# fabiocarrara/neural-ode-features

Measured on AMD Instinct MI355X. Metric: images/sec (fwd+adjoint) CIFAR-10 ODE-ResNet bs=128 at 1/2/4/8 GPU, higher is better.
Workload: dtype f32

## Files before the change

include/node_hip.h:

```cpp
#ifndef NODE_HIP_H
#define NODE_HIP_H

#include <stddef.h>
#include <stdint.h>

#ifdef __cplusplus
extern "C" {
#endif

#define NODE_ABI_VERSION 6

enum { NODE_METHOD_DOPRI5 = 0, NODE_METHOD_RK4 = 1 };

enum {
  NODE_OK = 0,
  NODE_ERR_NULL = -1,
  NODE_ERR_SHAPE = -2,
  NODE_ERR_UNSUPPORTED = -3,
  NODE_ERR_WORKSPACE = -4,
  NODE_ERR_MAX_STEPS = -5,
  NODE_ERR_NONFINITE = -6,
  NODE_ERR_DT_UNDERFLOW = -7,
  NODE_ERR_HIP = -8,
  NODE_ERR_ARG = -9
// ... 216 lines not shown
  const float* b1_n2_b;
  const float* b1_c2_w;
  const float* b1_ds_w;
  const float* b2_n1_w;
  const float* b2_n1_b;
  const float* b2_c1_w;
  const float* b2_n2_w;
  const float* b2_n2_b;
  const float* b2_c2_w;
  const float* b2_ds_w;
} node_stem_params;
typedef struct node_stem_grads {
  float* conv0_w; float* conv0_b;
  float* b1_n1_w; float* b1_n1_b; float* b1_c1_w; float* b1_n2_w; float* b1_n2_b; float* b1_c2_w; float* b1_ds_w;
  float* b2_n1_w; float* b2_n1_b; float* b2_c1_w; float* b2_n2_w; float* b2_n2_b; float* b2_c2_w; float* b2_ds_w;
} node_stem_grads;
size_t node_stem_workspace_bytes(const node_stem_shape* shape);
int node_stem_fwd(const node_stem_shape* shape, const node_stem_params* params, const float* x, float* out,
                  void* ws, size_t ws_bytes, void* stream);
int node_stem_bwd(const node_stem_shape* shape, const node_stem_params* params, const float* x, const float* grad_out,
                  const node_stem_grads* grads, void* ws, size_t ws_bytes, void* stream);
int node_stem_bwd_dx(const node_stem_shape* shape, const node_stem_params* params, const float* x, const float* grad_out,
                     const node_stem_grads* grads, float* d_x, void* ws, size_t ws_bytes, void* stream);
size_t node_stem_conv0_dgrad_workspace_bytes(const node_stem_shape* shape);
int node_stem_conv0_dgrad(const node_stem_shape* shape, const float* w0, const float* dy, float* d_x,
                          void* ws, size_t ws_bytes, void* stream);

typedef struct node_conv_geom {
  int32_t n, cin, cout, x_h, x_w, k, stride, pad;
} node_conv_geom;
size_t node_stem_conv_workspace_bytes(const node_conv_geom* g);
int node_stem_conv(const node_conv_geom* g, int what, const float* x, const float* w, const float* dy, float* result,
                   void* ws, size_t ws_bytes, void* stream);

typedef struct node_trunk_shape {
  int32_t n, channels, h, w, blocks;
  float eps;
} node_trunk_shape;
typedef struct node_trunk_block {
  const float* n1_w;
  const float* n1_b;
  const float* c1_w;
  const float* n2_w;
  const float* n2_b;
  const float* c2_w;
} node_trunk_block;
typedef struct node_trunk_block_grads {
  float* n1_w; float* n1_b; float* c1_w; float* n2_w; float* n2_b; float* c2_w;
} node_trunk_block_grads;
size_t node_trunk_workspace_bytes(const node_trunk_shape* shape, int keep_for_backward);
int node_trunk_fwd(const node_trunk_shape* shape, const node_trunk_block* blocks, const float* x, float* out, float* taps,
                   int keep_for_backward, void* ws, size_t ws_bytes, void* stream);
int node_trunk_bwd(const node_trunk_shape* shape, const node_trunk_block* blocks, const float* grad_out,
                   const node_trunk_block_grads* grads, float* d_x, void* ws, size_t ws_bytes, void* stream);

size_t node_retrieval_workspace_bytes(int nq, int nd, int d);
int node_retrieval_ap(int nq, int nd, int d, const float* q, const float* x, const int32_t* q_labels, const int32_t* x_labels,
                      int k, double* ap, double* ap_k, void* ws, size_t ws_bytes, void* stream);
int node_rank_ap(int nq, int nd, const float* scores, const int32_t* q_labels, const int32_t* x_labels, int k, double* ap,
                 double* ap_k, void* ws, size_t ws_bytes, void* stream);

typedef struct { int32_t fold; int32_t cls; float c; } node_svm_problem;
typedef struct { int32_t iterations; int32_t converged; double grad_ratio; } node_svm_result;
size_t node_svm_workspace_bytes(int n, int d, int p);
int node_svm_fit(int n, int d, int p, const float* x, const int32_t* labels, const int32_t* row_fold,
                 const node_svm_problem* problems, double eps, int max_iter, float* weights, node_svm_result* results, void* ws,
// ... 56 lines not shown
```

neural-ode-features_amd/_lib.py:

```python
from __future__ import annotations

import ctypes as C
import os

HERE = os.path.dirname(os.path.abspath(__file__))
LIB_PATH = os.path.join(HERE, 'csrc', 'libnode_hip.so')
LIB_DIAG_PATH = os.path.join(HERE, 'csrc', 'libnode_hip_diag.so')

NODE_ABI_VERSION = 6
METHOD_DOPRI5, METHOD_RK4 = 0, 1
METHODS = {'dopri5': METHOD_DOPRI5, 'rk4': METHOD_RK4}

ERRORS = {
    0: 'NODE_OK', -1: 'NODE_ERR_NULL', -2: 'NODE_ERR_SHAPE', -3: 'NODE_ERR_UNSUPPORTED',
    -4: 'NODE_ERR_WORKSPACE', -5: 'NODE_ERR_MAX_STEPS', -6: 'NODE_ERR_NONFINITE',
    -7: 'NODE_ERR_DT_UNDERFLOW', -8: 'NODE_ERR_HIP', -9: 'NODE_ERR_ARG',
}

EXPORTS = [
    'node_abi_version', 'node_last_error', 'node_param_count', 'node_workspace_bytes', 'node_solve_is_resident',
    'node_describe_dims',
    'node_odefunc_fwd', 'node_odefunc_vjp', 'node_solve_fwd', 'node_solve_adjoint',
    'node_backprop_workspace_bytes', 'node_solve_backprop',
    'node_head_fwd', 'node_head_bwd', 'node_gn_relu_fwd', 'node_gn_relu_bwd',
    'node_sgd_step', 'node_adam_step', 'node_profile_begin', 'node_profile_end',
    'node_conv3x3_w4_workspace_bytes', 'node_conv3x3_w4', 'node_w4_split3', 'node_w4_pair_stats',
    'node_stem_workspace_bytes', 'node_stem_fwd', 'node_stem_bwd', 'node_stem_conv_workspace_bytes', 'node_stem_conv',
    'node_stem_bwd_dx', 'node_stem_conv0_dgrad_workspace_bytes', 'node_stem_conv0_dgrad', 'node_attack_step', 'node_attack_judge',
    'node_head_loss_scratch_bytes', 'node_head_loss_fwd', 'node_head_loss_bwd',
    'node_flat_workspace_bytes', 'node_flat_begin', 'node_flat_stage', 'node_flat_scalar', 'node_flat_initial_step',
    'node_flat_finish_step', 'node_flat_status_read',
    'node_retrieval_workspace_bytes', 'node_retrieval_ap', 'node_rank_ap',
    'node_svm_workspace_bytes', 'node_svm_fit', 'node_svm_cv_score',
    'node_augment_batch',
    'node_imgconv_workspace_bytes', 'node_imgconv_fwd', 'node_imgconv_bwd',
    'node_trunk_workspace_bytes', 'node_trunk_fwd', 'node_trunk_bwd',
]


class NodeShape(C.Structure):
    _fields_ = [('n', C.c_int32), ('c', C.c_int32), ('h', C.c_int32), ('w', C.c_int32),
                ('groups', C.c_int32), ('eps', C.c_float)]


class NodeParams(C.Structure):
    _fields_ = [(k, C.c_void_p) for k in (
        'norm1_w', 'norm1_b', 'conv1_w', 'conv1_b', 'norm2_w', 'norm2_b',
        'conv2_w', 'conv2_b', 'norm3_w', 'norm3_b')]


WGRAD_KERNELS = ('W2_8', 'W2_4', 'W_8_8', 'W_16_2', 'W_4_4', 'T_8_8', 'T_16_4', 'T_7_7', 'T_4_4', 'P')
CONV_KERNELS = ('DIRECT_64', 'DIRECT_128', 'DIRECT_256', 'W1_64', 'W1_128', 'W1_256', 'W2_128')


class NodeDimsInfo(C.Structure):
    _fields_ = [(k, C.c_int32) for k in (
        'wgrad_kernel', 'conv_kernel', 'wino', 'bm', 's', 'csplit', 'mtiles', 'ntile', 'small', 'tiny', 'wino4', 'w4q',
        'wgrad_wino', 'wut', 'rb', 'nbands', 'nsplit', 'wgrad_pair')]


def describe_dims(n, c, h, w, groups=None, eps=1e-5):
# ... 42 lines not shown

class NodeAdamTensor(C.Structure):
    _fields_ = [('param', C.c_void_p), ('grad', C.c_void_p), ('exp_avg', C.c_void_p), ('exp_avg_sq', C.c_void_p),
                ('step', C.c_void_p), ('n', C.c_size_t)]


STEM_PARAM_FIELDS = ('conv0_w', 'conv0_b', 'b1_n1_w', 'b1_n1_b', 'b1_c1_w', 'b1_n2_w', 'b1_n2_b', 'b1_c2_w', 'b1_ds_w',
                     'b2_n1_w', 'b2_n1_b', 'b2_c1_w', 'b2_n2_w', 'b2_n2_b', 'b2_c2_w', 'b2_ds_w')


class NodeStemShape(C.Structure):
    _fields_ = [('n', C.c_int32), ('in_ch', C.c_int32), ('h', C.c_int32), ('w', C.c_int32), ('filters', C.c_int32),
                ('eps', C.c_float)]


class NodeStemParams(C.Structure):
    _fields_ = [(k, C.c_void_p) for k in STEM_PARAM_FIELDS]


TRUNK_BLOCK_FIELDS = ('n1_w', 'n1_b', 'c1_w', 'n2_w', 'n2_b', 'c2_w')


class NodeTrunkShape(C.Structure):
    _fields_ = [('n', C.c_int32), ('channels', C.c_int32), ('h', C.c_int32), ('w', C.c_int32), ('blocks', C.c_int32),
                ('eps', C.c_float)]


class NodeTrunkBlock(C.Structure):
    _fields_ = [(k, C.c_void_p) for k in TRUNK_BLOCK_FIELDS]


class NodeConvGeom(C.Structure):
    _fields_ = [(k, C.c_int32) for k in ('n', 'cin', 'cout', 'x_h', 'x_w', 'k', 'stride', 'pad')]


REDUCE_MEAN, REDUCE_SUM = 0, 1


class NodeHeadLoss(C.Structure):
    _fields_ = [('n', C.c_int32), ('c', C.c_int32), ('classes', C.c_int32), ('reduction', C.c_int32),
                ('pooled', C.c_void_p), ('weight', C.c_void_p), ('bias', C.c_void_p), ('target', C.c_void_p),
                ('logits', C.c_void_p), ('loss', C.c_void_p), ('stat', C.c_void_p), ('scratch', C.c_void_p)]


class NodeHeadLossGrad(C.Structure):
    _fields_ = [(k, C.c_void_p) for k in ('grad_loss', 'grad_logits', 'd_logits', 'd_pooled', 'd_weight', 'd_bias')]


class NodeFlatSeg(C.Structure):
    _fields_ = [('y', C.c_void_p), ('y1', C.c_void_p), ('k', C.c_void_p * 7), ('n', C.c_size_t)]


class NodeFlatSolve(C.Structure):
    _fields_ = [('nseg', C.c_int32), ('has_scalar', C.c_int32), ('seg', NodeFlatSeg * 3), ('rtol', C.c_float), ('atol', C.c_float),
                ('tsign', C.c_float), ('n_targets', C.c_int32), ('ws', C.c_void_p), ('ws_bytes', C.c_size_t)]


class NodeFlatStatus(C.Structure):
    _fields_ = [('done', C.c_int32), ('status', C.c_int32), ('steps', C.c_int32), ('accepted', C.c_int32), ('rejected', C.c_int32),
                ('t', C.c_double), ('dt', C.c_double), ('first_dt', C.c_double), ('scalar', C.c_float)]


FLAT_F0, FLAT_PROBE = -1, -2

AUG_CROP, AUG_JITTER, AUG_FLIP, AUG_NORM = 1, 2, 4, 8

# ... 75 lines not shown
    lib.node_head_fwd.argtypes = [P(NodeShape), vp, vp, vp, vp, vp, vp, vp]
    lib.node_head_bwd.restype = i32
    lib.node_head_bwd.argtypes = [P(NodeShape), vp, vp, vp, vp, vp, vp, vp, vp, vp, vp]
    lib.node_gn_relu_fwd.restype = i32
    lib.node_gn_relu_fwd.argtypes = [P(NodeShape), vp, vp, vp, i32, vp, vp, vp]
    lib.node_gn_relu_bwd.restype = i32
    lib.node_gn_relu_bwd.argtypes = [P(NodeShape), vp, vp, vp, vp, i32, vp, vp, vp, vp, vp]
    lib.node_sgd_step.restype = i32
    lib.node_sgd_step.argtypes = [P(NodeSgdTensor), i32, f32, f32, f32, f32, vp, vp]
    lib.node_adam_step.restype = i32
    lib.node_adam_step.argtypes = [P(NodeAdamTensor), i32, f32, f32, f32, f32, f32, f32, vp, vp]
    lib.node_profile_begin.restype = i32
    lib.node_profile_begin.argtypes = []
    lib.node_profile_end.restype = i32
    lib.node_profile_end.argtypes = [P(NodeProfile)]
    lib.node_conv3x3_w4_workspace_bytes.restype = sz
    lib.node_conv3x3_w4_workspace_bytes.argtypes = [P(NodeShape)]
    lib.node_w4_pair_stats.restype = i32
    lib.node_w4_pair_stats.argtypes = [P(C.c_int32)]
    lib.node_conv3x3_w4.restype = i32
    lib.node_conv3x3_w4.argtypes = [P(NodeShape), vp, i32, vp, vp, vp, sz, vp]
    lib.node_w4_split3.restype = i32
    lib.node_w4_split3.argtypes = [vp, vp, sz, vp]
    lib.node_stem_workspace_bytes.restype = sz
    lib.node_stem_workspace_bytes.argtypes = [P(NodeStemShape)]
    lib.node_stem_fwd.restype = i32
    lib.node_stem_fwd.argtypes = [P(NodeStemShape), P(NodeStemParams), vp, vp, vp, sz, vp]
    lib.node_stem_bwd.restype = i32
    lib.node_stem_bwd.argtypes = [P(NodeStemShape), P(NodeStemParams), vp, vp, P(NodeStemParams), vp, sz, vp]
    lib.node_stem_conv_workspace_bytes.restype = sz
    lib.node_stem_conv_workspace_bytes.argtypes = [P(NodeConvGeom)]
    lib.node_stem_conv.restype = i32
    lib.node_stem_conv.argtypes = [P(NodeConvGeom), i32, vp, vp, vp, vp, vp, sz, vp]
    lib.node_stem_bwd_dx.restype = i32
    lib.node_stem_bwd_dx.argtypes = [P(NodeStemShape), P(NodeStemParams), vp, vp, P(NodeStemParams), vp, vp, sz, vp]
    lib.node_stem_conv0_dgrad_workspace_bytes.restype = sz
    lib.node_stem_conv0_dgrad_workspace_bytes.argtypes = [P(NodeStemShape)]
    lib.node_stem_conv0_dgrad.restype = i32
    lib.node_stem_conv0_dgrad.argtypes = [P(NodeStemShape), vp, vp, vp, vp, sz, vp]
    lib.node_attack_step.restype = i32
    lib.node_attack_step.argtypes = [P(NodeAttack), vp, vp, vp, vp, vp, vp]
    lib.node_attack_judge.restype = i32
    lib.node_attack_judge.argtypes = [P(NodeAttack), i32, vp, vp, vp, vp, i32, i32, P(NodeAttackRecord), vp]
    lib.node_head_loss_scratch_bytes.restype = sz
    lib.node_head_loss_scratch_bytes.argtypes = [i32]
    lib.node_head_loss_fwd.restype = i32
    lib.node_head_loss_fwd.argtypes = [P(NodeHeadLoss), vp]
    lib.node_head_loss_bwd.restype = i32
    lib.node_head_loss_bwd.argtypes = [P(NodeHeadLoss), P(NodeHeadLossGrad), vp]
    lib.node_flat_workspace_bytes.restype = sz
    lib.node_flat_workspace_bytes.argtypes = [i32]
    lib.node_flat_begin.restype = i32
    lib.node_flat_begin.argtypes = [P(NodeFlatSolve), C.c_double, P(C.c_double), C.c_double, i32, vp]
    lib.node_flat_stage.restype = i32
    lib.node_flat_stage.argtypes = [P(NodeFlatSolve), i32, i32, P(C.c_void_p), vp, vp]
    lib.node_flat_scalar.restype = i32
    lib.node_flat_scalar.argtypes = [P(NodeFlatSolve), i32, vp, f32, i32, vp]
    lib.node_flat_initial_step.restype = i32
    lib.node_flat_initial_step.argtypes = [P(NodeFlatSolve), i32, vp]
    lib.node_flat_finish_step.restype = i32
    lib.node_flat_finish_step.argtypes = [P(NodeFlatSolve), i32, vp, vp]
    lib.node_flat_status_read.restype = i32
    lib.node_flat_status_read.argtypes = [P(NodeFlatSolve), P(NodeFlatStatus), vp]
    lib.node_retrieval_workspace_bytes.restype = sz
    lib.node_retrieval_workspace_bytes.argtypes = [i32, i32, i32]
    lib.node_retrieval_ap.restype = i32
# ... 34 lines not shown
```

neural-ode-features_amd/csrc/kernels_stem.hip:

```cpp
#include "stem.h"
#include <type_traits>

namespace node {

namespace {

typedef float f32x16 __attribute__((ext_vector_type(16)));
typedef __bf16 bf16x8 __attribute__((ext_vector_type(8)));
typedef __bf16 bf16x2 __attribute__((ext_vector_type(2)));
typedef float f32x2 __attribute__((ext_vector_type(2)));
typedef unsigned u32x4 __attribute__((ext_vector_type(4)));

__device__ __forceinline__ void split3(float x, bf16_t& h, bf16_t& m, bf16_t& l) {
  const __bf16 bh = (__bf16)x;
  const float r = x - (float)bh;
  const __bf16 bm = (__bf16)r;
  const float r2 = r - (float)bm;
  const __bf16 bl = (__bf16)r2;
  h = __builtin_bit_cast(bf16_t, bh);
  m = __builtin_bit_cast(bf16_t, bm);
  l = __builtin_bit_cast(bf16_t, bl);
}
__device__ __forceinline__ void split8(const float4& p, const float4& q, u32x4& hh, u32x4& mm, u32x4& ll) {
  const f32x2 v[4] = {{p.x, p.y}, {p.z, p.w}, {q.x, q.y}, {q.z, q.w}};
#pragma unroll
  for (int i = 0; i < 4; ++i) {
    const bf16x2 h = __builtin_convertvector(v[i], bf16x2);
    const f32x2 r = v[i] - __builtin_convertvector(h, f32x2);
    const bf16x2 m = __builtin_convertvector(r, bf16x2);
    const f32x2 r2 = r - __builtin_convertvector(m, f32x2);
    const bf16x2 l = __builtin_convertvector(r2, bf16x2);
    hh[i] = __builtin_bit_cast(unsigned, h);
    mm[i] = __builtin_bit_cast(unsigned, m);
// ... 544 lines not shown
    } else {
#pragma unroll
      for (int q = 0; q < 8; ++q) av[q] = make_float4(0.f, 0.f, 0.f, 0.f);
    }
    f32x16 acc;
#pragma unroll
    for (int i = 0; i < 16; ++i) acc[i] = 0.f;
#pragma unroll
    for (int q = 0; q < 8; ++q) {
      acc = __builtin_amdgcn_mfma_f32_32x32x2f32(av[q].x, b[4 * q], acc, 0, 0, 0);
      acc = __builtin_amdgcn_mfma_f32_32x32x2f32(av[q].y, b[4 * q + 1], acc, 0, 0, 0);
      acc = __builtin_amdgcn_mfma_f32_32x32x2f32(av[q].z, b[4 * q + 2], acc, 0, 0, 0);
      acc = __builtin_amdgcn_mfma_f32_32x32x2f32(av[q].w, b[4 * q + 3], acc, 0, 0, 0);
    }
    if (li < 28) {
#pragma unroll
      for (int i = 0; i < 16; ++i) P[(tile * 32 + 8 * (i >> 2) + 4 * hh + (i & 3)) * DG_PS + li] = acc[i];
    }
  }
  __syncthreads();
  for (int idx = t; idx < Cin * DG_TH * DG_TW; idx += 256) {
    const int xx = idx % DG_TW, yy = (idx / DG_TW) % DG_TH, ci = idx / (DG_TW * DG_TH);
    const int y = y0 + yy, x = x0 + xx;
    if (y >= H || x >= W) continue;
    float s = 0.f;
#pragma unroll
    for (int ky = 0; ky < 3; ++ky)
#pragma unroll
      for (int kx = 0; kx < 3; ++kx) s += P[((yy + 2 - ky) * DG_PW + xx + 2 - kx) * DG_PS + ci * 9 + ky * 3 + kx];
    dx[((size_t)(n * Cin + ci) * H + y) * W + x] = s;
  }
}

__device__ __forceinline__ void group_sums(float v, float* red, float* grp, int CB, int cpg, int t) {
  red[t] = v;
  __syncthreads();
  const int ngrp = CB / cpg;
  if (t < ngrp) {
    float s = 0.f;
    for (int j = 0; j < 256 / CB; ++j)
      for (int k = 0; k < cpg; ++k) s += red[j * CB + t * cpg + k];
    grp[t] = s;
  }
  __syncthreads();
}

__global__ __launch_bounds__(256) void k_stem_gn_fwd(const SGnArgs a) {
  extern __shared__ __align__(16) unsigned char smem[];
  const int t = threadIdx.x;
  const int CB = a.CB, HW = a.HW, C = a.C;
  float* tile = reinterpret_cast<float*>(smem);
  float* red = tile + (size_t)HW * CB;
  float* gmean = red + 256;
  float* grstd = gmean + 128;
  const int nblk = C / CB;
  const int n = blockIdx.x / nblk, c0 = (blockIdx.x - n * nblk) * CB;
  const int q4 = CB >> 2;
  const float* src = a.h + ((size_t)n * HW) * C + c0;
  for (int idx = t; idx < HW * q4; idx += 256) {
    const int px = idx / q4, q = idx - px * q4;
    *reinterpret_cast<float4*>(tile + px * CB + 4 * q) = *reinterpret_cast<const float4*>(src + (size_t)px * C + 4 * q);
  }
  __syncthreads();
  const int c = t & (CB - 1), pg = t / CB, PG = 256 / CB;
  const float inv_m = 1.f / (float)(a.cpg * HW);
  float s = 0.f;
  for (int px = pg; px < HW; px += PG) s += tile[px * CB + c];
  group_sums(s, red, gmean, CB, a.cpg, t);
  const float mean = gmean[c / a.cpg] * inv_m;
  float s2 = 0.f;
  for (int px = pg; px < HW; px += PG) {
    const float d = tile[px * CB + c] - mean;
    s2 += d * d;
  }
  group_sums(s2, red, grstd, CB, a.cpg, t);
  const int ngrp = CB / a.cpg;
  if (t < ngrp) {
    const float m = gmean[t] * inv_m, rs = rsqrtf(grstd[t] * inv_m + a.eps);
    float* st = a.stats + ((size_t)n * (C / a.cpg) + c0 / a.cpg + t) * 2;
    st[0] = m;
    st[1] = rs;
  }
  __syncthreads();
  if (t < ngrp) {
    const float m = gmean[t] * inv_m, rs = rsqrtf(grstd[t] * inv_m + a.eps);
    gmean[t] = m;
    grstd[t] = rs;
  }
  __syncthreads();
  const int q8 = CB >> 3;
  for (int idx = t; idx < HW * q8; idx += 256) {
    const int px = idx / q8, q = idx - px * q8;
    const float4 p0 = *reinterpret_cast<const float4*>(tile + px * CB + 8 * q);
    const float4 p1 = *reinterpret_cast<const float4*>(tile + px * CB + 8 * q + 4);
    float v[8] = {p0.x, p0.y, p0.z, p0.w, p1.x, p1.y, p1.z, p1.w};
#pragma unroll
    for (int k = 0; k < 8; ++k) {
      const int cc = 8 * q + k, g = cc / a.cpg;
      const float y = (v[k] - gmean[g]) * grstd[g] * a.gamma[c0 + cc] + a.beta[c0 + cc];
      v[k] = fmaxf(y, 0.f);
    }
    u32x4 hh, mm, ll;
    split8(make_float4(v[0], v[1], v[2], v[3]), make_float4(v[4], v[5], v[6], v[7]), hh, mm, ll);
    bf16_t* dst = a.a3 + ((size_t)n * HW + px) * C + c0 + 8 * q;
    *reinterpret_cast<u32x4*>(dst) = hh;
    *reinterpret_cast<u32x4*>(dst + a.a_plane) = mm;
    *reinterpret_cast<u32x4*>(dst + 2 * a.a_plane) = ll;
  }
}

template <bool SKIP>
__global__ __launch_bounds__(256) void k_stem_gn_bwd(const SGnArgs a) {
  extern __shared__ __align__(16) unsigned char smem[];
  const int CB = a.CB, HW = a.HW, C = a.C;
  float* txh = reinterpret_cast<float*>(smem);
  float* tdy = txh + (size_t)HW * CB;
  float* redA = tdy + (size_t)HW * CB;
  float* redB = redA + 256;
  float* gmean = redB + 256;
  float* grstd = gmean + 128;
  float* gs1 = grstd + 128;
  float* gs2 = gs1 + 128;
  const int t = threadIdx.x;
  const int nblk = C / CB;
  const int n = blockIdx.x / nblk, c0 = (blockIdx.x - n * nblk) * CB;
  const int q4 = CB >> 2;
  const float* sh = a.h + ((size_t)n * HW) * C + c0;
  const float* sd = a.da + ((size_t)n * HW) * C + c0;
  for (int idx = t; idx < HW * q4; idx += 256) {
    const int px = idx / q4, q = idx - px * q4;
    *reinterpret_cast<float4*>(txh + px * CB + 4 * q) = *reinterpret_cast<const float4*>(sh + (size_t)px * C + 4 * q);
    *reinterpret_cast<float4*>(tdy + px * CB + 4 * q) = *reinterpret_cast<const float4*>(sd + (size_t)px * C + 4 * q);
  }
  const int ngrp = CB / a.cpg;
  if (t < ngrp) {
    const float* st = a.stats + ((size_t)n * (C / a.cpg) + c0 / a.cpg + t) * 2;
    gmean[t] = st[0];
    grstd[t] = st[1];
  }
  __syncthreads();
  const int c = t & (CB - 1), pg = t / CB, PG = 256 / CB;
  const float mean = gmean[c / a.cpg], rstd = grstd[c / a.cpg], gam = a.gamma[c0 + c], bet = a.beta[c0 + c];
  float sA = 0.f, sB = 0.f;
  for (int px = pg; px < HW; px += PG) {
    const float xh = (txh[px * CB + c] - mean) * rstd;
    const float y = xh * gam + bet;
    const float dy = y > 0.f ? tdy[px * CB + c] : 0.f;
    txh[px * CB + c] = xh;
    tdy[px * CB + c] = dy;
    sA += dy;
    sB += dy * xh;
  }
  redA[t] = sA;
  redB[t] = sB;
  __syncthreads();
  if (t < CB) {
    float A = 0.f, B = 0.f;
    for (int j = 0; j < PG; ++j) { A += redA[j * CB + t]; B += redB[j * CB + t]; }
    a.gpart[((size_t)n * 2 + 0) * C + c0 + t] = B;
    a.gpart[((size_t)n * 2 + 1) * C + c0 + t] = A;
    redA[t] = A * gam;
    redB[t] = B * gam;
  }
  __syncthreads();
  if (t < ngrp) {
    float s1 = 0.f, s2 = 0.f;
    for (int k = 0; k < a.cpg; ++k) { s1 += redA[t * a.cpg + k]; s2 += redB[t * a.cpg + k]; }
    gs1[t] = s1;
    gs2[t] = s2;
  }
  __syncthreads();
  const float inv_m = 1.f / (float)(a.cpg * HW);
  const int q8 = CB >> 3;
  for (int idx = t; idx < HW * q8; idx += 256) {
    const int px = idx / q8, q = idx - px * q8;
    float v[8];
#pragma unroll
    for (int k = 0; k < 8; ++k) {
      const int cc = 8 * q + k, g = cc / a.cpg;
      const float xh = txh[px * CB + cc], dy = tdy[px * CB + cc];
      v[k] = grstd[g] * (dy * a.gamma[c0 + cc] - (gs1[g] + xh * gs2[g]) * inv_m);
    }
    const size_t o = ((size_t)n * HW + px) * C + c0 + 8 * q;
    if constexpr (SKIP) {
      const float4 k0 = *reinterpret_cast<const float4*>(a.skip + o), k1 = *reinterpret_cast<const float4*>(a.skip + o + 4);
      v[0] += k0.x; v[1] += k0.y; v[2] += k0.z; v[3] += k0.w;
      v[4] += k1.x; v[5] += k1.y; v[6] += k1.z; v[7] += k1.w;
    }
    const float4 p0 = make_float4(v[0], v[1], v[2], v[3]), p1 = make_float4(v[4], v[5], v[6], v[7]);
    if (a.dh) {
      *reinterpret_cast<float4*>(a.dh + o) = p0;
      *reinterpret_cast<float4*>(a.dh + o + 4) = p1;
    }
    if (a.dh3) {
      u32x4 hh, mm, ll;
      split8(p0, p1, hh, mm, ll);
      *reinterpret_cast<u32x4*>(a.dh3 + o) = hh;
      *reinterpret_cast<u32x4*>(a.dh3 + o + a.dh_plane) = mm;
      *reinterpret_cast<u32x4*>(a.dh3 + o + 2 * a.dh_plane) = ll;
    }
  }
}

__global__ __launch_bounds__(256) void k_stem_from_nchw(const float* __restrict__ src, float* __restrict__ dst, bf16_t* __restrict__ dst3,
                                                        size_t plane, int C, int HW) {
  __shared__ float tile[64][65];
  const int t = threadIdx.x;
  const int npb = (HW + 63) / 64, ncb = C / 64;
  const int n = blockIdx.x / (npb * ncb), rem = blockIdx.x - n * npb * ncb, cb = rem / npb, pb = rem - cb * npb;
  const int c0 = cb * 64, p0 = pb * 64;
  for (int idx = t; idx < 64 * 64; idx += 256) {
    const int cc = idx >> 6, pp = idx & 63;
    tile[cc][pp] = p0 + pp < HW ? src[((size_t)n * C + c0 + cc) * HW + p0 + pp] : 0.f;
  }
  __syncthreads();
  for (int idx = t; idx < 64 * 8; idx += 256) {
    const int pp = idx >> 3, q = idx & 7;
    if (p0 + pp >= HW) continue;
// ... 114 lines not shown
    const int o = t & 31, g = t >> 5;
    const size_t idx = (size_t)bx * 32 + o;
    if ((size_t)bx * 32 >= nout) return;
    const bool on = idx < nout;
    const float* src = j.slab + (on ? idx : 0);
    float acc = 0.f;
    int k = g;
    for (; k + 56 < j.ns; k += 64) {
      float v[8];
#pragma unroll
      for (int q = 0; q < 8; ++q) v[q] = src[(size_t)(k + 8 * q) * nout];
      acc += ((v[0] + v[1]) + (v[2] + v[3])) + ((v[4] + v[5]) + (v[6] + v[7]));
    }
    for (; k < j.ns; k += 8) acc += src[(size_t)k * nout];
    part[g >> 1][(g & 1) * 32 + o] = acc;
    __syncthreads();
    if (g != 0 || !on) return;
    const float sum = ((part[0][o] + part[0][32 + o]) + (part[1][o] + part[1][32 + o])) + ((part[2][o] + part[2][32 + o]) + (part[3][o] + part[3][32 + o]));
    if (j.kind == 1) {
      const int co = (int)(idx >> 5), kk = (int)(idx & 31);
      if (kk < j.Ci) j.out[co * j.Ci + kk] = sum;
      else if (kk == j.Ci) j.out2[co] = sum;
    } else {
      if (idx < (size_t)j.Co) j.out[idx] = sum;
      else j.out2[idx - j.Co] = sum;
    }
  }
}

}

static bool stem_ring() { return env_int("NODE_TUNE_STEM_RING", 1) != 0; }

void launch_stem_conv(const SConvArgs& a, hipStream_t s) {
  const int mt = a.cls_tile0[a.nclass];
  const int ntn = (a.Cout / 64) * ((a.mode == 0 && a.w2 != nullptr) ? 2 : 1);
#define STEM_CONV(KC, D)                                                                  \
  {                                                                                       \
    static bool attr[MAX_DEVICES] = {};                                                   \
    allow_full_lds(reinterpret_cast<const void*>(k_stem_conv<KC, D>), attr);              \
    const size_t lds = (size_t)(D + 1) * (3 * 128 + 3 * 64) * 2 * KC + 512;               \
    hipLaunchKernelGGL((k_stem_conv<KC, D>), dim3(mt * ntn), dim3(256), lds, s, a);        \
  }
  if (stem_ring()) STEM_CONV(32, STEM_RING_D)
  else STEM_CONV(64, 1)
#undef STEM_CONV
}

void launch_stem_wgrad(const SWgradArgs& a, hipStream_t s) {
  const int taps = a.KH * a.KW;
  const int grid = (a.Cin / 64) * (a.Cout / 64) * (taps == 9 ? 3 : 1) * a.nsplit;
  const int nimg = 1 + (taps == 9 ? 3 : 1) + (a.dy23 ? 1 : 0);
#define STEM_WG(T, EX, D)                                                                \
  {                                                                                       \
    static bool attr[MAX_DEVICES] = {};                                                   \
    allow_full_lds(reinterpret_cast<const void*>(k_stem_wgrad<T, EX, D>), attr);          \
    const size_t lds = (size_t)(D + 1) * nimg * 3 * 16 * 128;                             \
    hipLaunchKernelGGL((k_stem_wgrad<T, EX, D>), dim3(grid), dim3(256), lds, s, a);        \
  }
  if (stem_ring()) {
    if (taps == 9 && a.dy23) STEM_WG(3, true, STEM_RING_D)
    else if (taps == 9) STEM_WG(3, false, STEM_RING_D)
    else STEM_WG(1, false, STEM_RING_D)
  } else {
    if (taps == 9 && a.dy23) STEM_WG(3, true, 1)
    else if (taps == 9) STEM_WG(3, false, 1)
    else STEM_WG(1, false, 1)
  }
#undef STEM_WG
}

void launch_stem_conv0_fwd(const float* x, const float* w0t, const float* bias, float* h0, int N, int Cin, int H, int W, hipStream_t s) {
  const int rows = N * (H - 2) * (W - 2);
  hipLaunchKernelGGL(k_stem_conv0_fwd, dim3((rows + 127) / 128), dim3(256), 0, s, x, w0t, bias, h0, N, Cin, H, W);
}
void launch_stem_conv0_wgrad(const float* x, const float* dh0, float* slab, int N, int Cin, int H, int W, int nsplit, int rows_per_split,
                             hipStream_t s) {
  hipLaunchKernelGGL(k_stem_conv0_wgrad, dim3(nsplit), dim3(256), 0, s, x, dh0, slab, N, Cin, H, W, rows_per_split);
}
void launch_stem_conv0_dgrad(const float* dh0, const float* w0, float* dx, int N, int Cin, int H, int W, hipStream_t s) {
  const int tx = (W + DG_TW - 1) / DG_TW, ty = (H + DG_TH - 1) / DG_TH;
  hipLaunchKernelGGL(k_stem_conv0_dgrad, dim3((unsigned)(N * tx * ty)), dim3(256), 0, s, dh0, w0, dx, Cin, H, W, tx, ty);
}

int stem_gn_cb(int HW, int C, int cpg) {
  const size_t budget = 150 * 1024;
  int cb = 8;
  while (cb < cpg) cb *= 2;
  if (cb > C || cb > 128 || (size_t)HW * cb * 2 * sizeof(float) > budget) return 0;
  while (cb * 2 <= C && cb * 2 <= 128 && (size_t)HW * cb * 4 * sizeof(float) <= budget) cb *= 2;
  static const int cap = env_int("NODE_TUNE_STEM_GNCB", -1);
  while (cap > 0 && cb > cap && cb / 2 >= cpg && cb / 2 >= 8) cb /= 2;
  if (C % cb != 0 || cb % cpg != 0) return 0;
  return cb;
}
void launch_stem_gn_fwd(const SGnArgs& a, hipStream_t s) {
  static bool attr[MAX_DEVICES] = {};
  allow_full_lds(reinterpret_cast<const void*>(k_stem_gn_fwd), attr);
  hipLaunchKernelGGL(k_stem_gn_fwd, dim3(a.N * (a.C / a.CB)), dim3(256), ((size_t)a.HW * a.CB + 512) * sizeof(float), s, a);
}
void launch_stem_gn_bwd(const SGnArgs& a, hipStream_t s) {
  const dim3 grid(a.N * (a.C / a.CB));
  const size_t lds = ((size_t)2 * a.HW * a.CB + 1024) * sizeof(float);
  if (a.skip) {
    static bool attr[MAX_DEVICES] = {};
    allow_full_lds(reinterpret_cast<const void*>(k_stem_gn_bwd<true>), attr);
    hipLaunchKernelGGL(k_stem_gn_bwd<true>, grid, dim3(256), lds, s, a);
  } else {
    static bool attr[MAX_DEVICES] = {};
    allow_full_lds(reinterpret_cast<const void*>(k_stem_gn_bwd<false>), attr);
    hipLaunchKernelGGL(k_stem_gn_bwd<false>, grid, dim3(256), lds, s, a);
  }
}

void launch_stem_prep(const SPrepArgs& a0, hipStream_t s) {
  SPrepArgs a = a0;
  unsigned at = 0;
  for (int i = 0; i < 6; ++i) {
    a.blk0[i] = at;
    if (i < a.njobs) at += (unsigned)(((size_t)a.job[i].taps * a.job[i].Cout * a.job[i].Cin + 255) / 256);
  }
  a.blk0[6] = at; at += (28 * 64 + 255) / 256;
  a.blk0[7] = at; at += (unsigned)(((size_t)a.nzero * 3 * 4096 + 255) / 256);
  a.blk0[8] = at;
  hipLaunchKernelGGL(k_stem_prep, dim3(at), dim3(256), 0, s, a);
}
void launch_stem_from_nchw(const float* src, float* dst_nhwc, bf16_t* dst3, size_t plane, int N, int C, int HW, hipStream_t s) {
  hipLaunchKernelGGL(k_stem_from_nchw, dim3(N * (C / 64) * ((HW + 63) / 64)), dim3(256), 0, s, src, dst_nhwc, dst3, plane, C, HW);
}
void launch_stem_split(const float* src, bf16_t* dst3, size_t plane, size_t n, hipStream_t s) {
  hipLaunchKernelGGL(k_stem_split, dim3((unsigned)((n / 8 + 255) / 256)), dim3(256), 0, s, src, dst3, plane, n / 8);
}
void launch_stem_to_nchw(const float* src_nhwc, float* dst, int N, int C, int HW, hipStream_t s) {
  hipLaunchKernelGGL(k_stem_to_nchw, dim3(N * (C / 64) * ((HW + 63) / 64)), dim3(256), 0, s, src_nhwc, dst, C, HW);
}
void launch_stem_reduce(const SReduceArgs& a0, hipStream_t s) {
  SReduceArgs a = a0;
  unsigned at = 0;
  for (int i = 0; i < a.njobs; ++i) {
    const SReduceJob& j = a.job[i];
    a.blk0[i] = at;
    at += (unsigned)(j.kind == 0 ? j.Co * j.taps : j.kind == 1 ? 64 : (2 * j.Co + 31) / 32);
  }
  a.blk0[a.njobs] = at;
  if (at == 0) return;
// ... 5 lines not shown
```

neural-ode-features_amd/csrc/stem.h:

```cpp
#pragma once
#include "node_internal.h"

namespace node {

typedef unsigned short bf16_t;

struct SConvArgs {
  const bf16_t* in;
  size_t in_plane;
  int zero_row;
  const bf16_t* w;
  size_t w_plane;
  float* out;
  const float* res;
  const float* bias;
  int accumulate;
  const bf16_t* w2;
  size_t w2_plane;
  float* out2;
  const bf16_t* in2;
  int N, IH, IW;
  int OH, OW;
  int Cin, Cout;
  int KH, KW, sshift, pad;
  int mode;
  int nclass, step;
  int cls_py[4], cls_px[4], cls_h[4], cls_w[4];
  int cls_tile0[5];
  int cls_ntap[4];
  unsigned long long cls_taps[4];
};
void launch_stem_conv(const SConvArgs& a, hipStream_t s);

struct SWgradArgs {
  const bf16_t* dy3;
  size_t dy_plane;
  int dy_zero_row;
  const bf16_t* dy23;
  const bf16_t* in;
  size_t in_plane;
  int zero_row;
  float* slab;
  float* slab2;
  int N, IH, IW, OH, OW, Cin, Cout, KH, KW, stride, pad;
  int nsplit, rows_per_split;
};
void launch_stem_wgrad(const SWgradArgs& a, hipStream_t s);

void launch_stem_conv0_fwd(const float* x, const float* w0t , const float* bias, float* h0 , int N, int Cin,
                           int H, int W, hipStream_t s);
void launch_stem_conv0_wgrad(const float* x, const float* dh0, float* slab, int N, int Cin, int H, int W, int nsplit,
                             int rows_per_split, hipStream_t s);
void launch_stem_conv0_dgrad(const float* dh0, const float* w0, float* dx, int N, int Cin, int H, int W, hipStream_t s);

struct SGnArgs {
  const float* h;
  const float* gamma;
  const float* beta;
  float* stats;
  bf16_t* a3;
  size_t a_plane;
  const float* da;
  float* dh;
  bf16_t* dh3;
  size_t dh_plane;
  float* gpart;
// ... 26 lines not shown
```

neural-ode-features_amd/csrc/stem_api.hip:

```cpp
#include "host_common.h"
#include "stem.h"
#include "stem_plan.h"
#include "wino4.h"
#include <cstring>

using namespace node;

namespace {

inline int down2(int h) { return (h - 1) / 2 + 1; }

struct StemPlan {
  int N, Cin0, H, W, F;
  int H0, W0, H1, W1, H2, W2, R0, R1, R2;
  float eps;
  float* w0t;
  Filt c1, c2, d1, c3, c4, d2;
  float *h0, *h1, *s1, *x1, *h3, *s2, *outn;
  Trip a0, a1, a2, a3;
  float* stats[4];
  float *da3, *da2, *da1, *da0, *dh0;
  Trip g3, dh3t, dx1t, dh1t;
  float* gpart[4];
  Wg w4, w3, w2, w1, w0;
// ... 451 lines not shown
  const int XHW = g->x_h * g->x_w, YHW = p.YH * p.YW;
  SPrepArgs pa;
  memset(&pa, 0, sizeof(pa));
  if (what != 2) { pa.job[0] = {w, p.f.wf, p.f.wd, g->cout, g->cin, g->k * g->k}; pa.njobs = 1; }
  pa.zero[0] = p.xin.p + (size_t)p.xin.rows * p.xin.C; pa.zero_plane[0] = p.xin.plane; pa.zero_c[0] = p.xin.C;
  pa.zero[1] = p.dyt.p + (size_t)p.dyt.rows * p.dyt.C; pa.zero_plane[1] = p.dyt.plane; pa.zero_c[1] = p.dyt.C;
  pa.nzero = 2;
  launch_stem_prep(pa, st);
  if (what == 0) {
    launch_stem_from_nchw(x, nullptr, p.xin.p, p.xin.plane, g->n, g->cin, XHW, st);
    launch_stem_conv(conv_fwd_args(p.xin, p.f, p.resn, g->n, g->x_h, g->x_w, p.YH, p.YW, g->k, g->stride, g->pad), st);
    launch_stem_to_nchw(p.resn, result, g->n, g->cout, YHW, st);
  } else if (what == 1) {
    launch_stem_from_nchw(dy, nullptr, p.dyt.p, p.dyt.plane, g->n, g->cout, YHW, st);
    SConvArgs c = conv_dgrad_args(p.dyt, p.f, p.resn, g->n, p.YH, p.YW, g->x_h, g->x_w, g->k, g->stride, g->pad);
    if (g->k == 1 && g->stride == 2) {
      if (hipMemsetAsync(p.resn, 0, (size_t)g->n * XHW * g->cin * sizeof(float), st) != hipSuccess) return fail(NODE_ERR_HIP, "memset failed");
    }
    launch_stem_conv(c, st);
    launch_stem_to_nchw(p.resn, result, g->n, g->cin, XHW, st);
  } else {
    launch_stem_from_nchw(x, nullptr, p.xin.p, p.xin.plane, g->n, g->cin, XHW, st);
    launch_stem_from_nchw(dy, nullptr, p.dyt.p, p.dyt.plane, g->n, g->cout, YHW, st);
    launch_stem_wgrad(wgrad_args(p.dyt, nullptr, p.xin, p.wg, g->n, g->x_h, g->x_w, p.YH, p.YW, g->cin, g->cout, g->k, g->stride, g->pad), st);
    SReduceArgs ra;
    memset(&ra, 0, sizeof(ra));
    ra.job[0] = {p.wg.slab, result, nullptr, 0, p.wg.nsplit, g->cout, g->cin, g->k * g->k};
    ra.njobs = 1;
    launch_stem_reduce(ra, st);
  }
  return launch_ok("node_stem_conv");
}

}
```

Baseline: 28740.

## Batch GroupNorm tile loads, cache per-channel params in registers, pick conv stage count by occupancy

The stem GroupNorm kernels gain a templated path that issues several float4 global loads before writing them to LDS. The same path replaces divisions with shifts, keeps gamma/beta/mean/rstd in registers, and prefetches the skip tensor one iteration ahead. The stem conv launcher now queries the CU count and occupancy to pick a non-ring two-blocks-per-CU variant when the grid exceeds the CU count. New C entry points expose GN and the stage choice. These aim to raise memory-level parallelism and occupancy, at the cost of more registers and extra host-side queries on first use.

```diff
diff --git a/include/node_hip.h b/include/node_hip.h
--- a/include/node_hip.h
+++ b/include/node_hip.h
@@ -272,6 +272,15 @@
 size_t node_stem_conv_workspace_bytes(const node_conv_geom* g);
 int node_stem_conv(const node_conv_geom* g, int what, const float* x, const float* w, const float* dy, float* result,
                    void* ws, size_t ws_bytes, void* stream);
+int node_stem_conv_stages(const node_conv_geom* g, int what);
+
+typedef struct node_gn_geom {
+  int32_t n, c, hw;
+  float eps;
+} node_gn_geom;
+int node_stem_gn_block(const node_gn_geom* g);
+int node_stem_gn(const node_gn_geom* g, int what, const float* h, const float* gamma, const float* beta, float* stats,
+                 const float* da, const float* skip, uint16_t* out3, float* out, float* gpart, void* stream);
 
 typedef struct node_trunk_shape {
   int32_t n, channels, h, w, blocks;
diff --git a/neural-ode-features_amd/_lib.py b/neural-ode-features_amd/_lib.py
--- a/neural-ode-features_amd/_lib.py
+++ b/neural-ode-features_amd/_lib.py
@@ -26,7 +26,8 @@
     'node_sgd_step', 'node_adam_step', 'node_profile_begin', 'node_profile_end',
     'node_conv3x3_w4_workspace_bytes', 'node_conv3x3_w4', 'node_w4_split3', 'node_w4_pair_stats',
     'node_stem_workspace_bytes', 'node_stem_fwd', 'node_stem_bwd', 'node_stem_conv_workspace_bytes', 'node_stem_conv',
-    'node_stem_bwd_dx', 'node_stem_conv0_dgrad_workspace_bytes', 'node_stem_conv0_dgrad', 'node_attack_step', 'node_attack_judge',
+    'node_stem_bwd_dx', 'node_stem_conv0_dgrad_workspace_bytes', 'node_stem_conv0_dgrad', 'node_stem_gn_block', 'node_stem_gn', 'node_stem_conv_stages',
+    'node_attack_step', 'node_attack_judge',
     'node_head_loss_scratch_bytes', 'node_head_loss_fwd', 'node_head_loss_bwd',
     'node_flat_workspace_bytes', 'node_flat_begin', 'node_flat_stage', 'node_flat_scalar', 'node_flat_initial_step',
     'node_flat_finish_step', 'node_flat_status_read',
@@ -135,6 +136,10 @@
 
 class NodeConvGeom(C.Structure):
     _fields_ = [(k, C.c_int32) for k in ('n', 'cin', 'cout', 'x_h', 'x_w', 'k', 'stride', 'pad')]
+
+
+class NodeGnGeom(C.Structure):
+    _fields_ = [('n', C.c_int32), ('c', C.c_int32), ('hw', C.c_int32), ('eps', C.c_float)]
 
 
 REDUCE_MEAN, REDUCE_SUM = 0, 1
@@ -276,6 +281,12 @@
     lib.node_stem_conv_workspace_bytes.argtypes = [P(NodeConvGeom)]
     lib.node_stem_conv.restype = i32
     lib.node_stem_conv.argtypes = [P(NodeConvGeom), i32, vp, vp, vp, vp, vp, sz, vp]
+    lib.node_stem_gn_block.restype = i32
+    lib.node_stem_gn_block.argtypes = [P(NodeGnGeom)]
+    lib.node_stem_conv_stages.restype = i32
+    lib.node_stem_conv_stages.argtypes = [P(NodeConvGeom), i32]
+    lib.node_stem_gn.restype = i32
+    lib.node_stem_gn.argtypes = [P(NodeGnGeom), i32, vp, vp, vp, vp, vp, vp, vp, vp, vp, vp]
     lib.node_stem_bwd_dx.restype = i32
     lib.node_stem_bwd_dx.argtypes = [P(NodeStemShape), P(NodeStemParams), vp, vp, P(NodeStemParams), vp, vp, sz, vp]
     lib.node_stem_conv0_dgrad_workspace_bytes.restype = sz
diff --git a/neural-ode-features_amd/csrc/kernels_stem.hip b/neural-ode-features_amd/csrc/kernels_stem.hip
--- a/neural-ode-features_amd/csrc/kernels_stem.hip
+++ b/neural-ode-features_amd/csrc/kernels_stem.hip
@@ -1,4 +1,5 @@
 #include "stem.h"
+#include <atomic>
 #include <type_traits>
 
 namespace node {
@@ -609,6 +610,29 @@
   }
 }
 
+constexpr int GN_FILL = 8;
+template <int U>
+__device__ __forceinline__ void gn_fetch(float4 (&v)[U], const float* __restrict__ src, int base, int total, int qs, int C) {
+#pragma unroll
+  for (int u = 0; u < U; ++u) {
+    const int idx = min(base + 256 * u, total - 1);
+    const int px = idx >> qs, q = idx - (px << qs);
+    v[u] = *reinterpret_cast<const float4*>(src + (size_t)px * C + 4 * q);
+  }
+}
+template <int U>
+__device__ __forceinline__ void gn_pin(float4 (&v)[U]) {
+#pragma unroll
+  for (int u = 0; u < U; ++u) asm volatile("" : "+v"(v[u].x), "+v"(v[u].y), "+v"(v[u].z), "+v"(v[u].w));
+}
+template <int U>
+__device__ __forceinline__ void gn_put(float* tile, const float4 (&v)[U], int base, int total) {
+#pragma unroll
+  for (int u = 0; u < U; ++u) {
+    const int idx = base + 256 * u;
+    if (idx < total) *reinterpret_cast<float4*>(tile + 4 * idx) = v[u];
+  }
+}
 __device__ __forceinline__ void group_sums(float v, float* red, float* grp, int CB, int cpg, int t) {
   red[t] = v;
   __syncthreads();
@@ -622,6 +646,7 @@
   __syncthreads();
 }
 
+template <bool FED>
 __global__ __launch_bounds__(256) void k_stem_gn_fwd(const SGnArgs a) {
   extern __shared__ __align__(16) unsigned char smem[];
   const int t = threadIdx.x;
@@ -634,9 +659,19 @@
   const int n = blockIdx.x / nblk, c0 = (blockIdx.x - n * nblk) * CB;
   const int q4 = CB >> 2;
   const float* src = a.h + ((size_t)n * HW) * C + c0;
-  for (int idx = t; idx < HW * q4; idx += 256) {
-    const int px = idx / q4, q = idx - px * q4;
-    *reinterpret_cast<float4*>(tile + px * CB + 4 * q) = *reinterpret_cast<const float4*>(src + (size_t)px * C + 4 * q);
+  if constexpr (FED) {
+    const int qs = __builtin_ctz(q4), total = HW * q4;
+    for (int base = t; base < total; base += 256 * GN_FILL) {
+      float4 v[GN_FILL];
+      gn_fetch(v, src, base, total, qs, C);
+      gn_pin(v);
+      gn_put(tile, v, base, total);
+    }
+  } else {
+    for (int idx = t; idx < HW * q4; idx += 256) {
+      const int px = idx / q4, q = idx - px * q4;
+      *reinterpret_cast<float4*>(tile + px * CB + 4 * q) = *reinterpret_cast<const float4*>(src + (size_t)px * C + 4 * q);
+    }
   }
   __syncthreads();
   const int c = t & (CB - 1), pg = t / CB, PG = 256 / CB;
@@ -666,15 +701,26 @@
   }
   __syncthreads();
   const int q8 = CB >> 3;
+  const int q_own = t & (q8 - 1);
+  float r_gam[8], r_bet[8], r_mean[8], r_rstd[8];
+  if constexpr (FED) {
+#pragma unroll
+    for (int k = 0; k < 8; ++k) {
+      const int cc = 8 * q_own + k, g = cc / a.cpg;
+      r_gam[k] = a.gamma[c0 + cc]; r_bet[k] = a.beta[c0 + cc]; r_mean[k] = gmean[g]; r_rstd[k] = grstd[g];
+    }
+  }
   for (int idx = t; idx < HW * q8; idx += 256) {
-    const int px = idx / q8, q = idx - px * q8;
+    const int px = FED ? idx >> __builtin_ctz(q8) : idx / q8, q = FED ? q_own : idx - px * q8;
     const float4 p0 = *reinterpret_cast<const float4*>(tile + px * CB + 8 * q);
     const float4 p1 = *reinterpret_cast<const float4*>(tile + px * CB + 8 * q + 4);
     float v[8] = {p0.x, p0.y, p0.z, p0.w, p1.x, p1.y, p1.z, p1.w};
 #pragma unroll
     for (int k = 0; k < 8; ++k) {
       const int cc = 8 * q + k, g = cc / a.cpg;
-      const float y = (v[k] - gmean[g]) * grstd[g] * a.gamma[c0 + cc] + a.beta[c0 + cc];
+      const float mean_g = FED ? r_mean[k] : gmean[g], rstd_g = FED ? r_rstd[k] : grstd[g];
+      const float gam_c = FED ? r_gam[k] : a.gamma[c0 + cc], bet_c = FED ? r_bet[k] : a.beta[c0 + cc];
+      const float y = (v[k] - mean_g) * rstd_g * gam_c + bet_c;
       v[k] = fmaxf(y, 0.f);
     }
     u32x4 hh, mm, ll;
@@ -686,7 +732,7 @@
   }
 }
 
-template <bool SKIP>
+template <bool SKIP, bool FED>
 __global__ __launch_bounds__(256) void k_stem_gn_bwd(const SGnArgs a) {
   extern __shared__ __align__(16) unsigned char smem[];
   const int CB = a.CB, HW = a.HW, C = a.C;
@@ -704,10 +750,23 @@
   const int q4 = CB >> 2;
   const float* sh = a.h + ((size_t)n * HW) * C + c0;
   const float* sd = a.da + ((size_t)n * HW) * C + c0;
-  for (int idx = t; idx < HW * q4; idx += 256) {
-    const int px = idx / q4, q = idx - px * q4;
-    *reinterpret_cast<float4*>(txh + px * CB + 4 * q) = *reinterpret_cast<const float4*>(sh + (size_t)px * C + 4 * q);
-    *reinterpret_cast<float4*>(tdy + px * CB + 4 * q) = *reinterpret_cast<const float4*>(sd + (size_t)px * C + 4 * q);
+  if constexpr (FED) {
+    const int qs = __builtin_ctz(q4), total = HW * q4;
+    for (int base = t; base < total; base += 256 * (GN_FILL / 2)) {
+      float4 vh[GN_FILL / 2], vd[GN_FILL / 2];
+      gn_fetch(vh, sh, base, total, qs, C);
+      gn_fetch(vd, sd, base, total, qs, C);
+      gn_pin(vh);
+      gn_pin(vd);
+      gn_put(txh, vh, base, total);
+      gn_put(tdy, vd, base, total);
+    }
+  } else {
+    for (int idx = t; idx < HW * q4; idx += 256) {
+      const int px = idx / q4, q = idx - px * q4;
+      *reinterpret_cast<float4*>(txh + px * CB + 4 * q) = *reinterpret_cast<const float4*>(sh + (size_t)px * C + 4 * q);
+      *reinterpret_cast<float4*>(tdy + px * CB + 4 * q) = *reinterpret_cast<const float4*>(sd + (size_t)px * C + 4 * q);
+    }
   }
   const int ngrp = CB / a.cpg;
   if (t < ngrp) {
@@ -749,18 +808,47 @@
   __syncthreads();
   const float inv_m = 1.f / (float)(a.cpg * HW);
   const int q8 = CB >> 3;
+  const int q_own = t & (q8 - 1);
+  float r_gam[8], r_rstd[8], r_s1[8], r_s2[8];
+  if constexpr (FED) {
+#pragma unroll
+    for (int k = 0; k < 8; ++k) {
+      const int cc = 8 * q_own + k, g = cc / a.cpg;
+      r_gam[k] = a.gamma[c0 + cc]; r_rstd[k] = grstd[g]; r_s1[k] = gs1[g]; r_s2[k] = gs2[g];
+    }
+  }
+  float4 skip_next[2];
+  auto skip_fetch = [&](int idx) {
+    const size_t o = ((size_t)n * HW + (idx >> __builtin_ctz(q8))) * C + c0 + 8 * q_own;
+    skip_next[0] = *reinterpret_cast<const float4*>(a.skip + o);
+    skip_next[1] = *reinterpret_cast<const float4*>(a.skip + o + 4);
+  };
+  if constexpr (SKIP && FED)
+    if (t < HW * q8) skip_fetch(t);
   for (int idx = t; idx < HW * q8; idx += 256) {
-    const int px = idx / q8, q = idx - px * q8;
+    const int px = FED ? idx >> __builtin_ctz(q8) : idx / q8, q = FED ? q_own : idx - px * q8;
+    float4 skip_now[2];
+    if constexpr (SKIP && FED) {
+      skip_now[0] = skip_next[0]; skip_now[1] = skip_next[1];
+      skip_fetch(idx + 256 < HW * q8 ? idx + 256 : idx);
+    }
     float v[8];
 #pragma unroll
     for (int k = 0; k < 8; ++k) {
       const int cc = 8 * q + k, g = cc / a.cpg;
       const float xh = txh[px * CB + cc], dy = tdy[px * CB + cc];
-      v[k] = grstd[g] * (dy * a.gamma[c0 + cc] - (gs1[g] + xh * gs2[g]) * inv_m);
+      const float rstd_g = FED ? r_rstd[k] : grstd[g], s1_g = FED ? r_s1[k] : gs1[g], s2_g = FED ? r_s2[k] : gs2[g];
+      const float gam_c = FED ? r_gam[k] : a.gamma[c0 + cc];
+      v[k] = rstd_g * (dy * gam_c - (s1_g + xh * s2_g) * inv_m);
     }
     const size_t o = ((size_t)n * HW + px) * C + c0 + 8 * q;
     if constexpr (SKIP) {
-      const float4 k0 = *reinterpret_cast<const float4*>(a.skip + o), k1 = *reinterpret_cast<const float4*>(a.skip + o + 4);
+      float4 k0, k1;
+      if constexpr (FED) {
+        k0 = skip_now[0]; k1 = skip_now[1];
+      } else {
+        k0 = *reinterpret_cast<const float4*>(a.skip + o); k1 = *reinterpret_cast<const float4*>(a.skip + o + 4);
+      }
       v[0] += k0.x; v[1] += k0.y; v[2] += k0.z; v[3] += k0.w;
       v[4] += k1.x; v[5] += k1.y; v[6] += k1.z; v[7] += k1.w;
     }
@@ -941,18 +1029,66 @@
 
 static bool stem_ring() { return env_int("NODE_TUNE_STEM_RING", 1) != 0; }
 
+static int stem_device_cus() {
+  static std::atomic<int> cus_of[MAX_DEVICES];
+  int dev = 0;
+  if (hipGetDevice(&dev) != hipSuccess || dev < 0 || dev >= MAX_DEVICES) { (void)hipGetLastError(); return 0; }
+  int cus = cus_of[dev].load(std::memory_order_relaxed);
+  if (cus == 0) {
+    int n = 0;
+    if (hipDeviceGetAttribute(&n, hipDeviceAttributeMultiprocessorCount, dev) != hipSuccess) { (void)hipGetLastError(); n = -1; }
+    cus = n > 0 ? n : -1;
+    cus_of[dev].store(cus, std::memory_order_relaxed);
+  }
+  return cus > 0 ? cus : 0;
+}
+static bool stem_conv_two_fit() {
+  static std::atomic<int> fit_of[MAX_DEVICES];
+  int dev = 0;
+  if (hipGetDevice(&dev) != hipSuccess || dev < 0 || dev >= MAX_DEVICES) { (void)hipGetLastError(); return false; }
+  int fit = fit_of[dev].load(std::memory_order_relaxed);
+  if (fit == 0) {
+    static bool attr[MAX_DEVICES] = {};
+    allow_full_lds(reinterpret_cast<const void*>(k_stem_conv<32, 1>), attr);
+    int per_cu = 0;
+    const size_t lds = (size_t)2 * (3 * 128 + 3 * 64) * 2 * 32 + 512;
+    if (hipOccupancyMaxActiveBlocksPerMultiprocessor(&per_cu, reinterpret_cast<const void*>(k_stem_conv<32, 1>), 256, lds) != hipSuccess) {
+      (void)hipGetLastError();
+      per_cu = 0;
+    }
+    fit = per_cu >= 2 ? 1 : -1;
+    fit_of[dev].store(fit, std::memory_order_relaxed);
+  }
+  return fit > 0;
+}
+static bool stem_conv_two_per_cu(int grid) {
+  const int force = env_int("NODE_TUNE_STEM_CONV2", -1);
+  if (force >= 0) return force != 0;
+  const int cus = stem_device_cus();
+  return cus > 0 && grid > cus && stem_conv_two_fit();
+}
+
+static int stem_conv_grid(const SConvArgs& a) {
+  return a.cls_tile0[a.nclass] * (a.Cout / 64) * ((a.mode == 0 && a.w2 != nullptr) ? 2 : 1);
+}
+int stem_conv_stages(const SConvArgs& a) {
+  if (!stem_ring()) return 1;
+  return stem_conv_two_per_cu(stem_conv_grid(a)) ? 2 : STEM_RING_D + 1;
+}
 void launch_stem_conv(const SConvArgs& a, hipStream_t s) {
-  const int mt = a.cls_tile0[a.nclass];
-  const int ntn = (a.Cout / 64) * ((a.mode == 0 && a.w2 != nullptr) ? 2 : 1);
+  const int grid = stem_conv_grid(a);
 #define STEM_CONV(KC, D)                                                                  \
   {                                                                                       \
     static bool attr[MAX_DEVICES] = {};                                                   \
     allow_full_lds(reinterpret_cast<const void*>(k_stem_conv<KC, D>), attr);              \
     const size_t lds = (size_t)(D + 1) * (3 * 128 + 3 * 64) * 2 * KC + 512;               \
-    hipLaunchKernelGGL((k_stem_conv<KC, D>), dim3(mt * ntn), dim3(256), lds, s, a);        \
-  }
-  if (stem_ring()) STEM_CONV(32, STEM_RING_D)
-  else STEM_CONV(64, 1)
+    hipLaunchKernelGGL((k_stem_conv<KC, D>), dim3(grid), dim3(256), lds, s, a);            \
+  }
+  switch (stem_conv_stages(a)) {
+    case 1: STEM_CONV(64, 1) break;
+    case 2: STEM_CONV(32, 1) break;
+    default: STEM_CONV(32, STEM_RING_D)
+  }
 #undef STEM_CONV
 }
 
@@ -992,34 +1128,49 @@
   hipLaunchKernelGGL(k_stem_conv0_dgrad, dim3((unsigned)(N * tx * ty)), dim3(256), 0, s, dh0, w0, dx, Cin, H, W, tx, ty);
 }
 
+static bool stem_gn_fed() { return env_int("NODE_TUNE_STEM_GN", 1) != 0; }
 int stem_gn_cb(int HW, int C, int cpg) {
   const size_t budget = 150 * 1024;
   int cb = 8;
   while (cb < cpg) cb *= 2;
   if (cb > C || cb > 128 || (size_t)HW * cb * 2 * sizeof(float) > budget) return 0;
   while (cb * 2 <= C && cb * 2 <= 128 && (size_t)HW * cb * 4 * sizeof(float) <= budget) cb *= 2;
-  static const int cap = env_int("NODE_TUNE_STEM_GNCB", -1);
+  const int cap = env_int("NODE_TUNE_STEM_GNCB", -1);
   while (cap > 0 && cb > cap && cb / 2 >= cpg && cb / 2 >= 8) cb /= 2;
   if (C % cb != 0 || cb % cpg != 0) return 0;
   return cb;
 }
 void launch_stem_gn_fwd(const SGnArgs& a, hipStream_t s) {
-  static bool attr[MAX_DEVICES] = {};
-  allow_full_lds(reinterpret_cast<const void*>(k_stem_gn_fwd), attr);
-  hipLaunchKernelGGL(k_stem_gn_fwd, dim3(a.N * (a.C / a.CB)), dim3(256), ((size_t)a.HW * a.CB + 512) * sizeof(float), s, a);
+  const dim3 grid(a.N * (a.C / a.CB));
+  const size_t lds = ((size_t)a.HW * a.CB + 512) * sizeof(float);
+#define STEM_GN_FWD(FED)                                                                  \
+  {                                                                                       \
+    static bool attr[MAX_DEVICES] = {};                                                   \
+    allow_full_lds(reinterpret_cast<const void*>(k_stem_gn_fwd<FED>), attr);              \
+    hipLaunchKernelGGL(k_stem_gn_fwd<FED>, grid, dim3(256), lds, s, a);                   \
+  }
+  if (stem_gn_fed()) STEM_GN_FWD(true)
+  else STEM_GN_FWD(false)
+#undef STEM_GN_FWD
 }
 void launch_stem_gn_bwd(const SGnArgs& a, hipStream_t s) {
   const dim3 grid(a.N * (a.C / a.CB));
   const size_t lds = ((size_t)2 * a.HW * a.CB + 1024) * sizeof(float);
+#define STEM_GN_BWD(SKIP, FED)                                                            \
+  {                                                                                       \
+    static bool attr[MAX_DEVICES] = {};                                                   \
+    allow_full_lds(reinterpret_cast<const void*>(k_stem_gn_bwd<SKIP, FED>), attr);        \
+    hipLaunchKernelGGL((k_stem_gn_bwd<SKIP, FED>), grid, dim3(256), lds, s, a);           \
+  }
+  const bool fed = stem_gn_fed();
   if (a.skip) {
-    static bool attr[MAX_DEVICES] = {};
-    allow_full_lds(reinterpret_cast<const void*>(k_stem_gn_bwd<true>), attr);
-    hipLaunchKernelGGL(k_stem_gn_bwd<true>, grid, dim3(256), lds, s, a);
+    if (fed) STEM_GN_BWD(true, true)
+    else STEM_GN_BWD(true, false)
   } else {
-    static bool attr[MAX_DEVICES] = {};
-    allow_full_lds(reinterpret_cast<const void*>(k_stem_gn_bwd<false>), attr);
-    hipLaunchKernelGGL(k_stem_gn_bwd<false>, grid, dim3(256), lds, s, a);
-  }
+    if (fed) STEM_GN_BWD(false, true)
+    else STEM_GN_BWD(false, false)
+  }
+#undef STEM_GN_BWD
 }
 
 void launch_stem_prep(const SPrepArgs& a0, hipStream_t s) {
diff --git a/neural-ode-features_amd/csrc/stem.h b/neural-ode-features_amd/csrc/stem.h
--- a/neural-ode-features_amd/csrc/stem.h
+++ b/neural-ode-features_amd/csrc/stem.h
@@ -31,7 +31,7 @@
   unsigned long long cls_taps[4];
 };
 void launch_stem_conv(const SConvArgs& a, hipStream_t s);
-
+int stem_conv_stages(const SConvArgs& a);
 struct SWgradArgs {
   const bf16_t* dy3;
   size_t dy_plane;
diff --git a/neural-ode-features_amd/csrc/stem_api.hip b/neural-ode-features_amd/csrc/stem_api.hip
--- a/neural-ode-features_amd/csrc/stem_api.hip
+++ b/neural-ode-features_amd/csrc/stem_api.hip
@@ -507,4 +507,44 @@
   return launch_ok("node_stem_conv");
 }
 
-}
+static int check_gn_geom(const node_gn_geom* g) {
+  if (!g) return fail(NODE_ERR_NULL, "geometry is NULL");
+  if (g->n <= 0 || g->hw <= 0 || g->c < 64 || (g->c & (g->c - 1)) != 0) return fail(NODE_ERR_SHAPE, "bad GroupNorm geometry");
+  if ((size_t)g->n * g->hw * g->c >= ((size_t)1 << 31)) return fail(NODE_ERR_UNSUPPORTED, "stem tensors must stay under 2^31 elements");
+  if (stem_gn_cb(g->hw, g->c, g->c / 32) == 0) return fail(NODE_ERR_UNSUPPORTED, "the GroupNorm passes hold (sample, channel block) in LDS");
+  return NODE_OK;
+}
+
+int node_stem_gn_block(const node_gn_geom* g) {
+  if (check_gn_geom(g) != NODE_OK) return 0;
+  return stem_gn_cb(g->hw, g->c, g->c / 32);
+}
+
+int node_stem_conv_stages(const node_conv_geom* g, int what) {
+  if (check_geom(g) != NODE_OK || (what != 0 && what != 1)) return 0;
+  OnePlan p = make_one(g, nullptr);
+  return stem_conv_stages(what == 0 ? conv_fwd_args(p.xin, p.f, p.resn, g->n, g->x_h, g->x_w, p.YH, p.YW, g->k, g->stride, g->pad)
+                                    : conv_dgrad_args(p.dyt, p.f, p.resn, g->n, p.YH, p.YW, g->x_h, g->x_w, g->k, g->stride, g->pad));
+}
+
+int node_stem_gn(const node_gn_geom* g, int what, const float* h, const float* gamma, const float* beta, float* stats, const float* da,
+                 const float* skip, uint16_t* out3, float* out, float* gpart, void* stream) {
+  int rc = check_gn_geom(g);
+  if (rc != NODE_OK) return rc;
+  if (what != 0 && what != 1) return fail(NODE_ERR_ARG, "what must be 0 or 1");
+  if (!h || !gamma || !beta || !stats) return fail(NODE_ERR_NULL, "a required pointer is NULL");
+  if (what == 0 ? !out3 : (!da || !gpart || (!out && !out3))) return fail(NODE_ERR_NULL, "a required pointer is NULL");
+  hipStream_t st = (hipStream_t)stream;
+  SGnArgs a = gn_args(h, gamma, beta, stats, g->n, g->hw, g->c, g->eps);
+  const size_t plane = (size_t)g->n * g->hw * g->c;
+  if (what == 0) {
+    a.a3 = out3; a.a_plane = plane;
+    launch_stem_gn_fwd(a, st);
+  } else {
+    a.da = da; a.skip = skip; a.dh = out; a.dh3 = out3; a.dh_plane = plane; a.gpart = gpart;
+    launch_stem_gn_bwd(a, st);
+  }
+  return launch_ok("node_stem_gn");
+}
+
+}
```

Result: no change. 28950 (median of 6 runs) (+0.7%).
